# andrewcsmith/soundsym

Hardware: NVIDIA B200
Metric: dtw_cell_updates_per_s (higher is better)
Workload: dtype f16 (packed-half DP scan on f16 tensor-core costs; winners refined in f64)

## Files before the change

### soundsym_b200/csrc/dtw_h2.cu

```cuda
#include <algorithm>
#include <atomic>

#include "match.cuh"
#include "tc_common.cuh"

namespace ss {

int dtw_rescore_finalize(ss_dict* d, ss_queries* q, int k, int kp, uint32_t nslots, const uint32_t* d_slot_qid, double eps,
                         const float* d_max_na, const float* d_max_nb, const float* d_slot_max_na, int bound_mode, uint8_t* d_uncert_flag,
                         uint32_t* d_out_idx, double* d_out_dist);

int dtw_second_chance(ss_dict* d, ss_queries* q, int k, int kp, uint32_t nslots, const uint32_t* d_slot_qid, const unsigned long long* d_partial,
                      uint32_t nlists, const unsigned long long* d_thr, double eps, const float* d_max_na, const float* d_max_nb,
                      const float* d_slot_max_na, int bound_mode, uint8_t* d_uncert_flag, uint32_t* d_out_idx, double* d_out_dist);

constexpr int kH2Slots = 2;
constexpr int kH2SlotCols = 64;
constexpr int kH2DpWarps = 4 * kH2Slots;
constexpr int kH2DpThreads = kH2DpWarps * 32;
constexpr int kH2Threads = (kH2DpWarps + 1) * 32;
constexpr int kH2DescInt4 = 4;
constexpr int kH2In = 1, kH2Out = 2;
constexpr int kH2ARing = 32;
constexpr int kH2MaxLong = 2048;

struct H2Params {
    const unsigned char* a_blocks;
    const uint64_t* group_off;
    const uint32_t* group_len;
    const uint32_t* slot_len;
    uint32_t ngroups;
    const unsigned char* tiles;
    const int4* desc;
    const uint32_t* slice_tile;
    uint32_t nslices, slice_begin;
    unsigned long long* partial;
    uint32_t max_len;
    float inv_s;
    unsigned long long* thr;
    float* dbg;
    uint32_t dbg_nseg;
    __half2* bnd;
    uint32_t bnd_rows;
    float eta;
    unsigned long long* timeline;
};
__device__ __forceinline__ unsigned long long h2_now() {
    unsigned long long t;
    asm volatile("mov.u64 %0, %%globaltimer;" : "=l"(t));
    return t;
}

template <int N>
__device__ __forceinline__ void h2_ld(uint32_t taddr, __half2* v);
template <>
__device__ __forceinline__ void h2_ld<4>(uint32_t taddr, __half2* v) {
    uint32_t r[4];
    asm volatile("tcgen05.ld.sync.aligned.32x32b.x4.pack::16b.b32 {%0, %1, %2, %3}, [%4];\n" : "=r"(r[0]), "=r"(r[1]), "=r"(r[2]), "=r"(r[3]) : "r"(taddr));
#pragma unroll
    for (int i = 0; i < 4; i++) v[i] = *reinterpret_cast<__half2*>(&r[i]);
}
template <>
__device__ __forceinline__ void h2_ld<8>(uint32_t taddr, __half2* v) {
    uint32_t r[8];
    asm volatile("tcgen05.ld.sync.aligned.32x32b.x8.pack::16b.b32 {%0, %1, %2, %3, %4, %5, %6, %7}, [%8];\n"
                 : "=r"(r[0]), "=r"(r[1]), "=r"(r[2]), "=r"(r[3]), "=r"(r[4]), "=r"(r[5]), "=r"(r[6]), "=r"(r[7])
                 : "r"(taddr));
#pragma unroll
    for (int i = 0; i < 8; i++) v[i] = *reinterpret_cast<__half2*>(&r[i]);
}
template <>
__device__ __forceinline__ void h2_ld<16>(uint32_t taddr, __half2* v) {
    uint32_t r[16];
    asm volatile(
        "tcgen05.ld.sync.aligned.32x32b.x16.pack::16b.b32 {%0, %1, %2, %3, %4, %5, %6, %7, %8, %9, %10, %11, %12, %13, %14, %15}, [%16];\n"
        : "=r"(r[0]), "=r"(r[1]), "=r"(r[2]), "=r"(r[3]), "=r"(r[4]), "=r"(r[5]), "=r"(r[6]), "=r"(r[7]), "=r"(r[8]), "=r"(r[9]), "=r"(r[10]),
          "=r"(r[11]), "=r"(r[12]), "=r"(r[13]), "=r"(r[14]), "=r"(r[15])
        : "r"(taddr));
#pragma unroll
    for (int i = 0; i < 16; i++) v[i] = *reinterpret_cast<__half2*>(&r[i]);
}
template <int NG>
__device__ __forceinline__ void h2_ld_row(uint32_t taddr, __half2 (&v)[4 * NG]) {
    constexpr int N = 4 * NG;
    int done = 0;
    if constexpr (N >= 32) {
        h2_ld<16>(taddr, v);
        h2_ld<16>(taddr + 32, v + 16);
        done = 32;
    } else if constexpr (N >= 16) {
        h2_ld<16>(taddr, v);
        done = 16;
    }
    if constexpr ((N & 8) != 0) {
        h2_ld<8>(taddr + 2 * done, v + done);
        done += 8;
    }
    if constexpr ((N & 4) != 0) h2_ld<4>(taddr + 2 * done, v + done);
}

__device__ __forceinline__ __half2 h2_min3(__half2 a, __half2 b, __half2 c) { return __hmin2(__hmin2(a, b), c); }
__device__ __forceinline__ __half2 h2_inf() {
    const uint32_t bits = 0x7C007C00u;
    return *reinterpret_cast<const __half2*>(&bits);
}
__device__ __forceinline__ __half2 h2_zero() {
    const uint32_t bits = 0u;
    return *reinterpret_cast<const __half2*>(&bits);
}
__device__ __forceinline__ __half2 h2_combine(__half2 a, __half2 b) {
    const uint32_t r = __byte_perm(*reinterpret_cast<uint32_t*>(&a), *reinterpret_cast<uint32_t*>(&b), 0x7610);
    return *reinterpret_cast<const __half2*>(&r);
}
__device__ __forceinline__ int h2_len_of(const int4& sc, int e) { return (int)((((e < 4) ? (uint32_t)sc.x : (uint32_t)sc.y) >> (8 * (e & 3))) & 0xFFu); }
__device__ __forceinline__ int h2_seg_of(const int4& sa, const int4& sb, int e) {
    return e == 0 ? sa.x : e == 1 ? sa.y : e == 2 ? sa.z : e == 3 ? sa.w : e == 4 ? sb.x : e == 5 ? sb.y : e == 6 ? sb.z : sb.w;
}
__device__ __forceinline__ uint32_t h2_selp(uint32_t a, uint32_t b, int pick_a) {
    uint32_t r;
    asm("{\n.reg .pred q;\nsetp.ne.s32 q, %3, 0;\nselp.b32 %0, %1, %2, q;\n}\n" : "=r"(r) : "r"(a), "r"(b), "r"(pick_a));
    return r;
}
__device__ __forceinline__ __half2 h2_pick4(const __half2* v, int r) {
    const uint32_t v0 = *reinterpret_cast<const uint32_t*>(&v[0]), v1 = *reinterpret_cast<const uint32_t*>(&v[1]);
    const uint32_t v2 = *reinterpret_cast<const uint32_t*>(&v[2]), v3 = *reinterpret_cast<const uint32_t*>(&v[3]);
    const uint32_t lo = h2_selp(v1, v0, r & 1), hi = h2_selp(v3, v2, r & 1);
    const uint32_t o = h2_selp(hi, lo, r & 2);
    return *reinterpret_cast<const __half2*>(&o);
}

template <int NG>
__device__ __forceinline__ void h2_band(const __half2 (&tm0)[4 * NG], const __half2 (&tm1)[4 * NG], __half2 (&d)[4 * NG], __half2 dinit, __half2 (&c0l)[4]) {
    __half2 left0 = h2_inf(), diag0 = dinit, left1 = h2_inf();
#pragma unroll
    for (int j = 0; j < 4 * NG; j++) {
        const __half2 up0 = d[j];
        const __half2 c0 = __hadd2(tm0[j], h2_min3(left0, up0, diag0));
        const __half2 c1 = __hadd2(tm1[j], h2_min3(left1, c0, left0));
        diag0 = up0;
        left0 = c0;
        left1 = c1;
        d[j] = c1;
        if (j >= 4 * (NG - 1)) c0l[j - 4 * (NG - 1)] = c0;
    }
}
template <int NG>
__device__ __forceinline__ void h2_band_io(const __half2 (&tm0)[4 * NG], const __half2 (&tm1)[4 * NG], __half2 (&d)[4 * NG], __half2 l0, __half2 dg0,
                                           __half2 l1, __half2 (&c0l)[4], __half2& o0, __half2& o1) {
    __half2 left0 = l0, diag0 = dg0, left1 = l1;
#pragma unroll
    for (int j = 0; j < 4 * NG; j++) {
        const __half2 up0 = d[j];
        const __half2 c0 = __hadd2(tm0[j], h2_min3(left0, up0, diag0));
        const __half2 c1 = __hadd2(tm1[j], h2_min3(left1, c0, left0));
        diag0 = up0;
        left0 = c0;
        left1 = c1;
        d[j] = c1;
        if (j >= 4 * (NG - 1)) c0l[j - 4 * (NG - 1)] = c0;
    }
    o0 = left0, o1 = left1;
}
template <int NG>
__device__ __forceinline__ void h2_band_row_io(const __half2 (&tm)[4 * NG], __half2 (&d)[4 * NG], __half2 l0, __half2 dg0, __half2& o0) {
    __half2 left = l0, diag = dg0;
#pragma unroll
    for (int j = 0; j < 4 * NG; j++) {
        const __half2 up = d[j];
        const __half2 cur = __hadd2(tm[j], h2_min3(left, up, diag));
        diag = up;
        left = cur;
        d[j] = cur;
    }
    o0 = left;
}
template <int NG>
__device__ __forceinline__ void h2_band_row(const __half2 (&tm)[4 * NG], __half2 (&d)[4 * NG], __half2 dinit) {
    __half2 left = h2_inf(), diag = dinit;
#pragma unroll
    for (int j = 0; j < 4 * NG; j++) {
        const __half2 up = d[j];
        const __half2 cur = __hadd2(tm[j], h2_min3(left, up, diag));
        diag = up;
        left = cur;
        d[j] = cur;
    }
}

template <int NB, int NG>
__device__ __forceinline__ void h2_step2(TcCursor& cur, __half2 (&d)[NB][4 * NG], __half2 dinit, __half2 (&c0l)[NB][4]) {
    constexpr int kBandCols = kH2SlotCols / NB;
    cur.wait();
    const uint32_t taddr = cur.taddr;
    __half2 tm0[NB][4 * NG], tm1[NB][4 * NG];
#pragma unroll
    for (int b = 0; b < NB; b++) {
        h2_ld_row<NG>(taddr + b * kBandCols, tm0[b]);
        h2_ld_row<NG>(taddr + kTcN + b * kBandCols, tm1[b]);
    }
    tc_wait_ld();
    cur.release();
#pragma unroll
    for (int b = 0; b < NB; b++) h2_band<NG>(tm0[b], tm1[b], d[b], dinit, c0l[b]);
}

template <int NB, int NG>
__device__ __forceinline__ void h2_tile(uint32_t L, uint32_t lmin, uint32_t Lm, const int4& sc, TcCursor& cur, __half2 (&res)[NB]) {
    __half2 d[NB][4 * NG];
#pragma unroll
    for (int b = 0; b < NB; b++) {
#pragma unroll
        for (int j = 0; j < 4 * NG; j++) d[b][j] = h2_inf();
        res[b] = h2_inf();
    }
    __half2 dinit = h2_zero();
    const uint32_t nfull = L >> 1;
    const uint32_t ncap = min((lmin - 1) >> 1, nfull);
    uint32_t st = 0;
    if (st < ncap && cur.buf) {
        __half2 c0l[NB][4];
        h2_step2<NB, NG>(cur, d, dinit, c0l);
        dinit = h2_inf();
        st++;
    }
    if (st + 2 <= ncap) {
        const uint32_t full0 = cur.full, taddr0 = cur.taddr;
        uint32_t par = cur.par;
#pragma unroll 1
        for (; st + 2 <= ncap; st += 2) {
            __half2 c0l[NB][4];
            TcCursor c0 = {0u, par, full0, taddr0, cur.full_sum, cur.taddr_sum};
            h2_step2<NB, NG>(c0, d, dinit, c0l);
            TcCursor c1 = {1u, par, full0 + 8u, taddr0 + (uint32_t)kTcBufCols, cur.full_sum, cur.taddr_sum};
            h2_step2<NB, NG>(c1, d, h2_inf(), c0l);
            dinit = h2_inf();
            par ^= 1u;
        }
        cur.par = par;
    }
    if (st < ncap) {
        __half2 c0l[NB][4];
        h2_step2<NB, NG>(cur, d, dinit, c0l);
        dinit = h2_inf();
        st++;
    }
#pragma unroll 1
    for (; st < nfull; st++) {
        __half2 c0l[NB][4];
        h2_step2<NB, NG>(cur, d, dinit, c0l);
        dinit = h2_inf();
        const bool end0 = 2 * st + 1 == Lm, end1 = 2 * st + 2 == Lm;
#pragma unroll
        for (int b = 0; b < NB; b++) {
            const int ra = (h2_len_of(sc, 2 * b) - 1) & 3, rb = (h2_len_of(sc, 2 * b + 1) - 1) & 3;
            const __half2 e0 = h2_combine(h2_pick4(c0l[b], ra), h2_pick4(c0l[b], rb));
            const __half2 e1 = h2_combine(h2_pick4(&d[b][4 * (NG - 1)], ra), h2_pick4(&d[b][4 * (NG - 1)], rb));
            res[b] = end0 ? e0 : (end1 ? e1 : res[b]);
        }
    }
    if (L & 1) {
        constexpr int kBandCols = kH2SlotCols / NB;
        cur.wait();
        __half2 tm0[NB][4 * NG];
#pragma unroll
        for (int b = 0; b < NB; b++) h2_ld_row<NG>(cur.taddr + b * kBandCols, tm0[b]);
        tc_wait_ld();
        cur.release();
#pragma unroll
        for (int b = 0; b < NB; b++) {
            h2_band_row<NG>(tm0[b], d[b], dinit);
            const int ra = (h2_len_of(sc, 2 * b) - 1) & 3, rb = (h2_len_of(sc, 2 * b + 1) - 1) & 3;
            const __half2 e = h2_combine(h2_pick4(&d[b][4 * (NG - 1)], ra), h2_pick4(&d[b][4 * (NG - 1)], rb));
            res[b] = (L == Lm) ? e : res[b];
        }
    }
}

template <int NG, bool IN, bool OUT>
__device__ __forceinline__ void h2_tile_strip(uint32_t L, uint32_t lmin, uint32_t Lm, const int4& sc, TcCursor& cur, __half2* bnd, __half2& res) {
    constexpr uint32_t kStride = kH2DpThreads;
    __half2 d[4 * NG];
#pragma unroll
    for (int j = 0; j < 4 * NG; j++) d[j] = h2_inf();
    res = h2_inf();
    __half2 prev_b = IN ? h2_inf() : h2_zero();
    const uint32_t nfull = L >> 1;
    const uint32_t ncap = OUT ? nfull : min((lmin - 1) >> 1, nfull);
    const int ra = (h2_len_of(sc, 0) - 1) & 3, rb = (h2_len_of(sc, 1) - 1) & 3;
#pragma unroll 1
    for (uint32_t st = 0; st < nfull; st++) {
        __half2 b0 = h2_inf(), b1 = h2_inf();
        if (IN) b0 = bnd[(size_t)(2 * st) * kStride], b1 = bnd[(size_t)(2 * st + 1) * kStride];
        cur.wait();
        const uint32_t taddr = cur.taddr;
        __half2 tm0[4 * NG], tm1[4 * NG], c0l[4], o0, o1;
        h2_ld_row<NG>(taddr, tm0);
        h2_ld_row<NG>(taddr + kTcN, tm1);
        tc_wait_ld();
        cur.release();
        h2_band_io<NG>(tm0, tm1, d, b0, prev_b, b1, c0l, o0, o1);
        prev_b = IN ? b1 : h2_inf();
        if (OUT) {
            bnd[(size_t)(2 * st) * kStride] = o0;
            bnd[(size_t)(2 * st + 1) * kStride] = o1;
        } else if (st >= ncap) {
            const bool end0 = 2 * st + 1 == Lm, end1 = 2 * st + 2 == Lm;
            const __half2 e0 = h2_combine(h2_pick4(c0l, ra), h2_pick4(c0l, rb));
            const __half2 e1 = h2_combine(h2_pick4(&d[4 * (NG - 1)], ra), h2_pick4(&d[4 * (NG - 1)], rb));
            res = end0 ? e0 : (end1 ? e1 : res);
        }
    }
    if (L & 1) {
        __half2 b0 = h2_inf();
        if (IN) b0 = bnd[(size_t)(L - 1) * kStride];
        cur.wait();
        __half2 tm0[4 * NG], o0;
        h2_ld_row<NG>(cur.taddr, tm0);
        tc_wait_ld();
        cur.release();
        h2_band_row_io<NG>(tm0, d, b0, prev_b, o0);
        if (OUT) {
            bnd[(size_t)(L - 1) * kStride] = o0;
        } else {
            const __half2 e = h2_combine(h2_pick4(&d[4 * (NG - 1)], ra), h2_pick4(&d[4 * (NG - 1)], rb));
            res = (L == Lm) ? e : res;
        }
    }
// ... 97 lines not shown
#pragma unroll
        for (int s = 0; s < KP; s++) list[s * kH2DpThreads] = 0xFFFFFFFFFFFFFFFFull;
        const unsigned long long thr0 = __ldcg(p.thr + g * kTcM + m);
        unsigned long long worst = thr0;
        int cnt = 0, wpos = 0;
        const uint32_t lane_addr = tmem_base + ((uint32_t)(q * 32) << 16) + slot * kH2SlotCols;
        const uint32_t Lm = p.slot_len[g * kTcM + m];
        TcCursor cur;
        cur.init(s32(t_full), lane_addr);
        const int4* dp = p.desc + ((size_t)t0 * kH2Slots + slot) * kH2DescInt4;
        int4 na = make_int4(0, 0, 0, 0), nb = na, nc = na;
        if (ntiles) na = __ldg(dp), nb = __ldg(dp + 1), nc = __ldg(dp + 2);
        for (uint32_t n = 0; n < ntiles; n++) {
            const int4 sa = na, sb = nb, sc = nc;
            dp += kH2Slots * kH2DescInt4;
            if (n + 1 < ntiles) na = __ldg(dp), nb = __ldg(dp + 1), nc = __ldg(dp + 2);
            const int ng = sc.z;
            __half2 res[NB];
            if constexpr (NB == 1) {
                switch (ng) {
                    case 5: h2_tile<1, 5>(L, lmin, Lm, sc, cur, res); break;
                    case 6: h2_tile<1, 6>(L, lmin, Lm, sc, cur, res); break;
                    case 7: h2_tile<1, 7>(L, lmin, Lm, sc, cur, res); break;
                    default: h2_tile<1, 8>(L, lmin, Lm, sc, cur, res); break;
                }
            } else if constexpr (NB == 2) {
                if (ng == 3) h2_tile<2, 3>(L, lmin, Lm, sc, cur, res);
                else h2_tile<2, 4>(L, lmin, Lm, sc, cur, res);
            } else {
                if (ng == 1) h2_tile<4, 1>(L, lmin, Lm, sc, cur, res);
                else h2_tile<4, 2>(L, lmin, Lm, sc, cur, res);
            }
            if (tl && threadIdx.x == 0 && n + 1 == (ntiles + 1) / 2) tl[6] = h2_now();
            if (Lm) {
#pragma unroll
                for (int b = 0; b < NB; b++) {
#pragma unroll
                    for (int hsel = 0; hsel < 2; hsel++) {
                        const int e = 2 * b + hsel;
                        const int seg = h2_seg_of(sa, sb, e);
                        if (seg >= 0) {
                            const float v = hsel ? __high2float(res[b]) : __low2float(res[b]);
                            const float dist = __fdividef(v * p.inv_s, (float)(Lm + (uint32_t)h2_len_of(sc, e)));
                            const unsigned long long key = ((unsigned long long)tc_f2ord(dist) << 32) | (uint32_t)seg;
                            if (key < worst && dist == dist) {
                                const bool full = cnt == KP;
                                list[(full ? wpos : cnt) * kH2DpThreads] = key;
                                cnt += full ? 0 : 1;
                                if (cnt == KP) {
                                    tc_list_max<KP, kH2DpThreads>(list, worst, wpos);
                                    worst = worst < thr0 ? worst : thr0;
                                }
                            }
                            if constexpr (DBG) p.dbg[(size_t)(g * kTcM + m) * p.dbg_nseg + seg] = dist;
                        }
                    }
                }
            }
        }
        tc_sort_list<KP, kH2DpThreads>(list, cnt);
        worst = list[(KP - 1) * kH2DpThreads];
        worst = worst < thr0 ? worst : thr0;
        asm volatile("bar.sync 1, %0;" ::"n"(kH2DpThreads) : "memory");
        if (tl && threadIdx.x == 0) tl[2] = h2_now(), tl[5] = clock64() - tl[5];
        if (slot == 0) {
            const unsigned long long* other = list + kTcM;
            for (int s = 0; s < KP; s++) {
                const unsigned long long key = other[s * kH2DpThreads];
                if (key >= worst) break;
                tc_insert_key<KP, kH2DpThreads>(list, worst, key);
                worst = worst < thr0 ? worst : thr0;
            }
            const unsigned long long kept_worst = list[(KP - 1) * kH2DpThreads];
            if (kept_worst != 0xFFFFFFFFFFFFFFFFull && kept_worst < thr0) atomicMin(p.thr + g * kTcM + m, kept_worst);
            unsigned long long* out = p.partial + ((size_t)slice * p.ngroups * kTcM + (size_t)g * kTcM + m) * KP;
#pragma unroll
            for (int s = 0; s < KP; s++) out[s] = list[s * kH2DpThreads];
        }
    }
    if constexpr (NB != 1) asm volatile("griddepcontrol.wait;" ::: "memory");
    tc_fence_before();
    __syncthreads();
    if (warp == kH2DpWarps) {
        tc_fence_after();
        asm volatile("tcgen05.dealloc.cta_group::1.sync.aligned.b32 %0, %1;" ::"r"(tmem_base), "r"(512u) : "memory");
    }
    if (tl && threadIdx.x == 0) tl[3] = h2_now();
}

template <int KP, int NB, bool DBG = false>
__global__ void __launch_bounds__(kH2Threads, 1) k_dtw_scan_h2_long(const H2Params p) {
    extern __shared__ unsigned char smem_raw[];
    unsigned char* smem = smem_raw + ((128u - (s32(smem_raw) & 127u)) & 127u);
    unsigned char* sA = smem;
    unsigned char* sB = smem + (size_t)kH2ARing * kTcATileBytes;
    uint64_t* bars = reinterpret_cast<uint64_t*>(sB + kTcStages * kTcBTileBytes);
    uint64_t* a_full = bars;
    uint64_t* a_empty = bars + 4;
    uint64_t* b_full = bars + 8;
    uint64_t* b_empty = bars + 12;
    uint64_t* t_full = bars + 16;
    uint64_t* t_empty = bars + 18;
    uint32_t* tmem_slot = reinterpret_cast<uint32_t*>(bars + 20);
    unsigned long long* topk = reinterpret_cast<unsigned long long*>(bars + 32);

    const int warp = threadIdx.x >> 5, lane = threadIdx.x & 31;
    const uint32_t g = blockIdx.x / p.nslices, slice = p.slice_begin + blockIdx.x % p.nslices;
    asm volatile("griddepcontrol.launch_dependents;" ::: "memory");
    const uint32_t glen = p.group_len[g];
    const uint32_t L = glen & 0xFFFFu, lmin = glen >> 16;
    const uint32_t t0 = p.slice_tile[slice], t1 = p.slice_tile[slice + 1];
    const uint32_t ntiles = t1 - t0;

    if (threadIdx.x == 0) {
        for (int s = 0; s < 4; s++) mb_init(&a_full[s], 1), mb_init(&a_empty[s], 1);
        for (int s = 0; s < kTcStages; s++) mb_init(&b_full[s], 1), mb_init(&b_empty[s], 1);
        for (int s = 0; s < 2; s++) mb_init(&t_full[s], 1), mb_init(&t_empty[s], kH2DpWarps);
        asm volatile("fence.mbarrier_init.release.cluster;" ::: "memory");
    }
    if (warp == kH2DpWarps) {
        asm volatile("tcgen05.alloc.cta_group::1.sync.aligned.shared::cta.b32 [%0], %1;" ::"r"(s32(tmem_slot)), "r"(512u) : "memory");
        asm volatile("tcgen05.relinquish_alloc_permit.cta_group::1.sync.aligned;" ::: "memory");
    }
    tc_fence_before();
    __syncthreads();
    tc_fence_after();
    const uint32_t tmem_base = *tmem_slot;
    if (warp == kH2DpWarps) {
        if (lane == 0 && ntiles) {
            const uint32_t bars_s = s32(bars), sA_s = s32(sA), sB_s = s32(sB);
            const uint32_t a_full_s = bars_s, a_empty_s = bars_s + 32, b_full_s = bars_s + 64, b_empty_s = bars_s + 96, t_full_s = bars_s + 128,
                           t_empty_s = bars_s + 144;
            const uint32_t npieces = (L + 7) >> 3;
            const bool streaming = npieces > 4;
            const uint32_t total_pieces = streaming ? ntiles * npieces : npieces;
            const unsigned char* a_src = p.a_blocks + p.group_off[g];
            auto load_piece = [&](uint32_t n) {
                const uint32_t pc = n % npieces, slot = streaming ? (n & 3u) : pc;
                const uint32_t rows = min(8u, L - 8u * pc);
                mbs_expect_tx(a_full_s + 8 * slot, rows * kTcATileBytes);
                tmas_g2s(sA_s + slot * 8 * kTcATileBytes, a_src + (size_t)pc * 8 * kTcATileBytes, rows * kTcATileBytes, a_full_s + 8 * slot);
            };
            for (uint32_t n = 0; n < total_pieces && n < 4; n++) load_piece(n);
            const unsigned char* tile_src = p.tiles + (size_t)t0 * kTcBTileBytes;
            for (uint32_t n = 0; n < ntiles && n < (uint32_t)kTcStages; n++) {
                mbs_expect_tx(b_full_s + 8 * n, kTcBTileBytes);
                tmas_g2s(sB_s + n * kTcBTileBytes, tile_src + (size_t)n * kTcBTileBytes, kTcBTileBytes, b_full_s + 8 * n);
            }
            tile_src += (size_t)kTcStages * kTcBTileBytes;
            const uint32_t idesc = (0u << 4) | ((uint32_t)(kTcN >> 3) << 17) | ((uint32_t)(kTcM >> 4) << 24);
            uint32_t cnt = 0, stage = 0, sphase = 0, use_n = 0;
            for (uint32_t n = 0; n < ntiles; n++) {
                mbs_wait_sleep(b_full_s + 8 * stage, sphase);
                const uint64_t bdesc = tc_smem_desc_s<kTcN>(sB_s + stage * kTcBTileBytes);
                for (uint32_t pc = 0; pc < npieces; pc++, use_n++) {
                    const uint32_t slot = streaming ? (use_n & 3u) : pc;
                    if (streaming && use_n >= 1 && use_n + 3 < total_pieces) {
                        mbs_wait_sleep(a_empty_s + 8 * ((use_n - 1) & 3u), ((use_n - 1) >> 2) & 1);
                        load_piece(use_n + 3);
                    }
                    if (streaming || n == 0) mbs_wait_sleep(a_full_s + 8 * slot, streaming ? ((use_n >> 2) & 1) : 0u);
                    const uint64_t adesc0 = tc_smem_desc_s<kTcM>(sA_s + slot * 8 * kTcATileBytes);
                    const uint32_t rows = min(8u, L - 8u * pc);
                    for (uint32_t r = 0; r < rows; r += 2, cnt++) {
                        const uint32_t buf = cnt & 1;
                        if (cnt >= 2) mbs_wait_sleep(t_empty_s + 8 * buf, ((cnt >> 1) - 1) & 1);
// ... 229 lines not shown
        for (int slot = 0; slot < kH2Slots; slot++) {
            int segs[8] = {-1, -1, -1, -1, -1, -1, -1, -1}, whole[4] = {0, 0, 0, 0};
            uint32_t lens[2] = {0, 0};
            for (int e = 0; e < 2 * nb; e++) {
                const size_t pos = (size_t)slot * 2 * nb + e;
                if (pos < take) {
                    segs[e] = (int)order[o + pos];
                    lens[e >> 2] |= (uint32_t)len_of(order[o + pos]) << (8 * (e & 3));
                    if (e < 4) whole[e] = len_of(order[o + pos]);
                }
            }
            desc.push_back(make_int4(segs[0], segs[1], segs[2], segs[3]));
            desc.push_back(make_int4(segs[4], segs[5], segs[6], segs[7]));
            desc.push_back(make_int4((int)lens[0], (int)lens[1], ng, 0));
            desc.push_back(make_int4(whole[0], whole[1], whole[2], whole[3]));
        }
        push_tile(nb, ng, (24u + 16u * (uint32_t)(nb * ng)) * (nb == 4 ? 3u : 2u) / 2u, false);
        o += take;
    }
    while (cur_kind < 4) {
        d->h2_first_tile[cur_kind == 1 ? 1 : 2] = (uint32_t)tile_nb.size();
        cur_kind *= 2;
    }
    d->h2_first_tile[3] = (uint32_t)tile_nb.size();
    const uint32_t ntiles = (uint32_t)tile_nb.size();
    d->h2_ntiles = ntiles;
    d->h2_slices.clear();
    if (!ntiles) return SS_OK;
    SS_TRY(upload(ctx, d->d_h2_desc, desc.data(), desc.size()));
    DevBuf<uint8_t> d_nb;
    SS_TRY(upload(ctx, d_nb, tile_nb.data(), tile_nb.size()));
    SS_CUDA(ctx, d->d_h2_tiles.reserve((size_t)ntiles * kTcBTileBytes / 2));
    k_h2_dict_tiles<<<ntiles, kTcN, 0, ctx->stream>>>(d->d_mfcc.p, d->d_off.p, d->c, d->d_mu.p, d->d_h2_desc.p, d_nb.p, ntiles, d->tc_nb_scale,
                                                     reinterpret_cast<unsigned char*>(d->d_h2_tiles.p));
    SS_LAUNCHED(ctx);
    SS_CUDA(ctx, cudaStreamSynchronize(ctx->stream));
    float S = 1.0f;
    while (S * d->tc_max_nb > 4096.f) S *= 0.5f;
    while (S * d->tc_max_nb < 2048.f && S < 64.f) S *= 2.0f;
    d->h2_s0 = S;
    d->h2_s = S;
    d->h2_bmax = d->tc_max_abs;
    {
        DevBuf<uint32_t> d_n;
        SS_CUDA(ctx, d_n.reserve(1));
        k_h2_nsmid<<<1, 1, 0, ctx->stream>>>(d_n.p);
        SS_LAUNCHED(ctx);
        SS_CUDA(ctx, cudaMemcpyAsync(&d->h2_nsmid, d_n.p, sizeof(uint32_t), cudaMemcpyDeviceToHost, ctx->stream));
        SS_CUDA(ctx, cudaStreamSynchronize(ctx->stream));
    }
    d->h2_ready = true;
    return SS_OK;
}

static void h2_cost_scale(ss_dict* d, const ss_queries* q) {
    float S = d->h2_s0;
    for (uint64_t l = 64; l < (uint64_t)d->max_len + q->max_len && S > 1.0f / 65536.f; l *= 2) S *= 0.5f;
    d->h2_s = S;
}

static int h2_queries_build(ss_dict* d, ss_queries* q) {
    ss_ctx* ctx = q->ctx;
    h2_cost_scale(d, q);
    if (q->h2_built && q->h2_dict_serial == d->tc_serial && q->h2_s_built == d->h2_s) return SS_OK;
    if (!q->tc_grouped) SS_TRY(dtw_tc_queries_group(q));
    SS_CUDA(ctx, q->d_h2_a.reserve(std::max<uint64_t>(q->tc_a_bytes, 16)));
    SS_CUDA(ctx, q->d_tc_slot_max_na.reserve(std::max<size_t>((size_t)q->tc_ngroups * kTcM, 1)));
    SS_CUDA(ctx, q->d_uncert_flag.reserve(std::max<size_t>(q->nq, 1)));
    SS_CUDA(ctx, q->d_tc_max_norm.reserve(1));
    SS_CUDA(ctx, cudaMemsetAsync(q->d_tc_max_norm.p, 0, sizeof(float), ctx->stream));
    if (q->tc_ngroups) {
        SS_CUDA(ctx, cudaMemsetAsync(q->d_tc_slot_max_na.p, 0, (size_t)q->tc_ngroups * kTcM * sizeof(float), ctx->stream));
        k_tc_query_tiles<<<dim3(q->tc_ngroups, q->max_len), kTcM, 0, ctx->stream>>>(q->d_mfcc.p, q->d_off.p, q->c, d->d_mu.p, q->d_tc_group_len.p,
                                                                 q->d_tc_group_off.p, q->d_tc_qid.p, d->tc_nb_scale, d->h2_s, q->d_h2_a.p,
                                                                 q->d_tc_max_norm.p, q->d_tc_slot_max_na.p);
        SS_LAUNCHED(ctx);
    }
    q->h2_built = true;
    q->h2_dict_serial = d->tc_serial;
    q->h2_s_built = d->h2_s;
    return SS_OK;
}

template <int KP, int NB, bool DBG, bool LONG>
static int h2_launch_kind(ss_ctx* ctx, H2Params p, uint32_t slice_begin, uint32_t nslices, size_t smem, bool dependent) {
    if (!nslices) return SS_OK;
    p.slice_begin = slice_begin;
    p.nslices = nslices;
    auto kern = LONG ? k_dtw_scan_h2_long<KP, NB, DBG> : k_dtw_scan_h2<KP, NB, DBG>;
    SS_CUDA(ctx, cudaFuncSetAttribute(kern, cudaFuncAttributeMaxDynamicSharedMemorySize, (int)smem));
    cudaLaunchConfig_t cfg = {};
    cfg.gridDim = dim3(p.ngroups * nslices);
    cfg.blockDim = dim3(kH2Threads);
    cfg.dynamicSmemBytes = smem;
    cfg.stream = ctx->stream;
    cudaLaunchAttribute attr[1];
    attr[0].id = cudaLaunchAttributeProgrammaticStreamSerialization;
    attr[0].val.programmaticStreamSerializationAllowed = 1;
    cfg.attrs = attr;
    cfg.numAttrs = dependent ? 1 : 0;
    SS_CUDA(ctx, cudaLaunchKernelEx(&cfg, kern, p));
    SS_LAUNCHED(ctx);
    return SS_OK;
}

static double h2_eta(const ss_dict* d) { return (13.0 * (double)d->h2_bmax + 4.0) * 5.9604644775390625e-08  / (double)d->h2_s; }

struct H2Plan {
    H2Params p;
    uint32_t kind_begin[4];
    uint32_t nslots;
    size_t smem;
    bool use_long;
};
constexpr int kH2Waves = 16;
constexpr int kH2Kp = 8;

static int h2_plan(ss_dict* d, ss_queries* q, int kp, H2Plan* plan) {
    ss_ctx* ctx = d->ctx;
    const uint32_t nslots = q->tc_ngroups * kTcM;
    if (d->h2_slices.size() > 64 && !d->h2_slices.count(q->tc_ngroups)) {
        SS_CUDA(ctx, cudaStreamSynchronize(ctx->stream));
        d->h2_slices.clear();
    }
    std::unique_ptr<ss_dict::H2Slices>& sl = d->h2_slices[q->tc_ngroups];
    if (!sl) {
        sl.reset(new ss_dict::H2Slices());
        const uint32_t want = std::max<uint32_t>(1, std::min<uint32_t>(((uint32_t)ctx->sm_count * kH2Waves + q->tc_ngroups - 1) / q->tc_ngroups,
                                                                       std::max<uint32_t>((uint32_t)ctx->sm_count, d->h2_ntiles / 12)));
        std::vector<uint32_t> st;
        uint64_t total = 0;
        for (uint32_t f : d->h_h2_tile_cost) total += f;
        const uint64_t per0 = std::max<uint64_t>(1, (total + want - 1) / want);
        int last_kind = -1, nkinds = 0;
        for (int kind = 0; kind < 3; kind++)
            if (d->h2_first_tile[kind + 1] > d->h2_first_tile[kind]) last_kind = kind, nkinds++;
        if (nkinds < 2) last_kind = -1;
        for (int kind = 0; kind < 3; kind++) {
            sl->kind_slice[kind] = (uint32_t)st.size();
            const uint64_t per = kind == last_kind ? std::max<uint64_t>(1, per0 / 2) : per0;
            uint64_t acc = per;
            for (uint32_t t = d->h2_first_tile[kind]; t < d->h2_first_tile[kind + 1]; t++) {
                if (acc >= per && !d->h_h2_tile_cont[t]) st.push_back(t), acc = 0;
                acc += d->h_h2_tile_cost[t];
            }
        }
        sl->kind_slice[3] = (uint32_t)st.size();
        st.push_back(d->h2_ntiles);
        SS_TRY(upload(ctx, sl->d_slice_tile, st.data(), st.size()));
    }
    const uint32_t nslices = sl->kind_slice[3];
    SS_CUDA(ctx, d->d_tc_partial.reserve((size_t)nslices * nslots * kp));
    SS_CUDA(ctx, d->d_cand_idx.reserve((size_t)nslots * kp));
    SS_CUDA(ctx, d->d_cand_adist.reserve((size_t)nslots * kp));
    if (!d->ev_scan0) {
        SS_CUDA(ctx, cudaEventCreate(&d->ev_scan0));
        SS_CUDA(ctx, cudaEventCreate(&d->ev_scan1));
    }
    H2Params& p = plan->p;
    p.a_blocks = q->d_h2_a.p;
    p.group_off = q->d_tc_group_off.p;
    p.group_len = q->d_tc_group_len.p;
    p.slot_len = q->d_tc_slot_len.p;
    p.ngroups = q->tc_ngroups;
    p.tiles = reinterpret_cast<const unsigned char*>(d->d_h2_tiles.p);
    p.desc = d->d_h2_desc.p;
    p.slice_tile = sl->d_slice_tile.p;
    p.nslices = nslices;
    p.slice_begin = 0;
    p.partial = d->d_tc_partial.p;
    p.max_len = q->max_len;
    p.inv_s = 1.0f / d->h2_s;
    SS_CUDA(ctx, d->d_h2_thr.reserve(std::max<uint32_t>(nslots, 1)));
    SS_CUDA(ctx, cudaMemsetAsync(d->d_h2_thr.p, 0xFF, (size_t)nslots * sizeof(unsigned long long), ctx->stream));
    p.thr = d->d_h2_thr.p;
    p.dbg = nullptr;
    p.dbg_nseg = 0;
    for (int i = 0; i < 4; i++) plan->kind_begin[i] = sl->kind_slice[i];
    plan->nslots = nslots;
    plan->use_long = d->h2_has_strips || q->max_len > (uint32_t)kTcMaxLen;
    p.bnd = nullptr;
    p.bnd_rows = 0;
    p.eta = 0.f;
    p.timeline = nullptr;
    if (plan->use_long) {
        if (d->h2_has_strips) {
            p.bnd_rows = (q->max_len + 1) & ~1u;
            SS_CUDA(ctx, d->d_h2_bnd.reserve((size_t)d->h2_nsmid * p.bnd_rows * kH2DpThreads));
            p.bnd = d->d_h2_bnd.p;
        }
        p.eta = (float)h2_eta(d) * 1.0001f;
        plan->smem = (size_t)kH2ARing * kTcATileBytes + kTcStages * kTcBTileBytes + 32 * 8 + (size_t)kp * kH2DpThreads * 8 + 1024;
    } else {
        plan->smem = (size_t)q->max_len * kTcATileBytes + kTcStages * kTcBTileBytes + 32 * 8 + (size_t)kp * kH2DpThreads * 8 + 1024;
    }
    return SS_OK;
}

template <int KP, bool DBG, bool LONG>
// ... 93 lines not shown
```

Before: 9146 billion.

## Add two-pipe H2 DTW scan kernel with split TMEM loads and register rebalancing

Adds a new kernel variant that runs two independent MMA/DP pipelines per CTA. Each pipeline has its own producer warp, B-tile stages and TMEM buffer, and the tiles of a slice are interleaved across the two pipes. DP warps now use a simple single-buffer cursor. Their TMEM row loads are split so the first half of the band is computed while the second half is still loading, and the buffer is released earlier. setmaxnreg shifts registers from producer warps to DP warps. The kernel is chosen for KP=8 with NB of 1 or 2. It aims to hide MMA and TMEM-load latency behind the scalar half2 DP recurrence, at the cost of more threads, more shared memory and a per-CTA merge of more top-k lists.

Measured after the change: 10250 billion, median of 6. 12.1% higher.

```diff
diff --git a/soundsym_b200/csrc/dtw_h2.cu b/soundsym_b200/csrc/dtw_h2.cu
--- a/soundsym_b200/csrc/dtw_h2.cu
+++ b/soundsym_b200/csrc/dtw_h2.cu
@@ -1,5 +1,6 @@
 #include <algorithm>
 #include <atomic>
+#include <type_traits>
 
 #include "match.cuh"
 #include "tc_common.cuh"
@@ -23,6 +24,12 @@
 constexpr int kH2In = 1, kH2Out = 2;
 constexpr int kH2ARing = 32;
 constexpr int kH2MaxLong = 2048;
+constexpr int kH2Pipes = 2;
+constexpr int kH2PDpWarps = kH2Pipes * kH2DpWarps;
+constexpr int kH2PDpThreads = kH2PDpWarps * 32;
+constexpr int kH2PThreads = (kH2PDpWarps + 4) * 32;
+constexpr int kH2PRegsDp = 112, kH2PRegsProd = 32;
+static_assert(kH2PDpThreads * kH2PRegsDp + 128 * kH2PRegsProd == kH2PThreads * 96, "setmaxnreg budget must match the launch pool");
 
 struct H2Params {
     const unsigned char* a_blocks;
@@ -187,25 +194,95 @@
     }
 }
 
-template <int NB, int NG>
-__device__ __forceinline__ void h2_step2(TcCursor& cur, __half2 (&d)[NB][4 * NG], __half2 dinit, __half2 (&c0l)[NB][4]) {
+template <int NG, int J0, int J1>
+__device__ __forceinline__ void h2_band_cols(const __half2* tm0, const __half2* tm1, __half2 (&d)[4 * NG], __half2& left0, __half2& diag0,
+                                             __half2& left1, __half2 (&c0l)[4]) {
+#pragma unroll
+    for (int j = J0; j < J1; j++) {
+        const __half2 up0 = d[j];
+        const __half2 c0 = __hadd2(tm0[j - J0], h2_min3(left0, up0, diag0));
+        const __half2 c1 = __hadd2(tm1[j - J0], h2_min3(left1, c0, left0));
+        diag0 = up0;
+        left0 = c0;
+        left1 = c1;
+        d[j] = c1;
+        if (j >= 4 * (NG - 1)) c0l[j - 4 * (NG - 1)] = c0;
+    }
+}
+
+struct H2PipeCursor {
+    uint32_t par, full, taddr;
+    __device__ __forceinline__ void wait() const {
+        mb_wait_addr(full, par);
+        tc_fence_after();
+    }
+    __device__ __forceinline__ void release() {
+        tc_fence_before();
+        mb_arrive_elect(full + 16);
+        par ^= 1u;
+    }
+};
+
+template <int NB, int NG, class Cur>
+__device__ __forceinline__ void h2_step2(Cur& cur, __half2 (&d)[NB][4 * NG], __half2 dinit, __half2 (&c0l)[NB][4]) {
     constexpr int kBandCols = kH2SlotCols / NB;
     cur.wait();
     const uint32_t taddr = cur.taddr;
-    __half2 tm0[NB][4 * NG], tm1[NB][4 * NG];
-#pragma unroll
-    for (int b = 0; b < NB; b++) {
-        h2_ld_row<NG>(taddr + b * kBandCols, tm0[b]);
-        h2_ld_row<NG>(taddr + kTcN + b * kBandCols, tm1[b]);
-    }
-    tc_wait_ld();
-    cur.release();
-#pragma unroll
-    for (int b = 0; b < NB; b++) h2_band<NG>(tm0[b], tm1[b], d[b], dinit, c0l[b]);
-}
-
-template <int NB, int NG>
-__device__ __forceinline__ void h2_tile(uint32_t L, uint32_t lmin, uint32_t Lm, const int4& sc, TcCursor& cur, __half2 (&res)[NB]) {
+    if constexpr (std::is_same<Cur, H2PipeCursor>::value && NB == 1) {
+        static_assert(NG >= 5, "NB = 1 tiles have 5..8 column groups");
+        __half2 left0 = h2_inf(), diag0 = dinit, left1 = h2_inf();
+        {
+            __half2 a0[16], a1[16];
+            h2_ld_row<4>(taddr, a0);
+            h2_ld_row<4>(taddr + kTcN, a1);
+            tc_wait_ld();
+            h2_band_cols<NG, 0, 16>(a0, a1, d[0], left0, diag0, left1, c0l[0]);
+        }
+        __half2 b0[4 * (NG - 4)], b1[4 * (NG - 4)];
+        h2_ld_row<NG - 4>(taddr + 32, b0);
+        h2_ld_row<NG - 4>(taddr + kTcN + 32, b1);
+        tc_wait_ld();
+        cur.release();
+        h2_band_cols<NG, 16, 4 * NG>(b0, b1, d[0], left0, diag0, left1, c0l[0]);
+    } else if constexpr (std::is_same<Cur, H2PipeCursor>::value) {
+        constexpr int H = NB / 2;
+        {
+            __half2 tm0[H][4 * NG], tm1[H][4 * NG];
+#pragma unroll
+            for (int b = 0; b < H; b++) {
+                h2_ld_row<NG>(taddr + b * kBandCols, tm0[b]);
+                h2_ld_row<NG>(taddr + kTcN + b * kBandCols, tm1[b]);
+            }
+            tc_wait_ld();
+#pragma unroll
+            for (int b = 0; b < H; b++) h2_band<NG>(tm0[b], tm1[b], d[b], dinit, c0l[b]);
+        }
+        __half2 tm0[H][4 * NG], tm1[H][4 * NG];
+#pragma unroll
+        for (int b = 0; b < H; b++) {
+            h2_ld_row<NG>(taddr + (H + b) * kBandCols, tm0[b]);
+            h2_ld_row<NG>(taddr + kTcN + (H + b) * kBandCols, tm1[b]);
+        }
+        tc_wait_ld();
+        cur.release();
+#pragma unroll
+        for (int b = 0; b < H; b++) h2_band<NG>(tm0[b], tm1[b], d[H + b], dinit, c0l[H + b]);
+    } else {
+        __half2 tm0[NB][4 * NG], tm1[NB][4 * NG];
+#pragma unroll
+        for (int b = 0; b < NB; b++) {
+            h2_ld_row<NG>(taddr + b * kBandCols, tm0[b]);
+            h2_ld_row<NG>(taddr + kTcN + b * kBandCols, tm1[b]);
+        }
+        tc_wait_ld();
+        cur.release();
+#pragma unroll
+        for (int b = 0; b < NB; b++) h2_band<NG>(tm0[b], tm1[b], d[b], dinit, c0l[b]);
+    }
+}
+
+template <int NB, int NG, class Cur>
+__device__ __forceinline__ void h2_tile(uint32_t L, uint32_t lmin, uint32_t Lm, const int4& sc, Cur& cur, __half2 (&res)[NB]) {
     __half2 d[NB][4 * NG];
 #pragma unroll
     for (int b = 0; b < NB; b++) {
@@ -217,32 +294,41 @@
     const uint32_t nfull = L >> 1;
     const uint32_t ncap = min((lmin - 1) >> 1, nfull);
     uint32_t st = 0;
-    if (st < ncap && cur.buf) {
-        __half2 c0l[NB][4];
-        h2_step2<NB, NG>(cur, d, dinit, c0l);
-        dinit = h2_inf();
-        st++;
-    }
-    if (st + 2 <= ncap) {
-        const uint32_t full0 = cur.full, taddr0 = cur.taddr;
-        uint32_t par = cur.par;
+    if constexpr (std::is_same<Cur, H2PipeCursor>::value) {
 #pragma unroll 1
-        for (; st + 2 <= ncap; st += 2) {
+        for (; st < ncap; st++) {
             __half2 c0l[NB][4];
-            TcCursor c0 = {0u, par, full0, taddr0, cur.full_sum, cur.taddr_sum};
-            h2_step2<NB, NG>(c0, d, dinit, c0l);
-            TcCursor c1 = {1u, par, full0 + 8u, taddr0 + (uint32_t)kTcBufCols, cur.full_sum, cur.taddr_sum};
-            h2_step2<NB, NG>(c1, d, h2_inf(), c0l);
+            h2_step2<NB, NG>(cur, d, dinit, c0l);
             dinit = h2_inf();
-            par ^= 1u;
-        }
-        cur.par = par;
-    }
-    if (st < ncap) {
-        __half2 c0l[NB][4];
-        h2_step2<NB, NG>(cur, d, dinit, c0l);
-        dinit = h2_inf();
-        st++;
+        }
+    } else {
+        if (st < ncap && cur.buf) {
+            __half2 c0l[NB][4];
+            h2_step2<NB, NG>(cur, d, dinit, c0l);
+            dinit = h2_inf();
+            st++;
+        }
+        if (st + 2 <= ncap) {
+            const uint32_t full0 = cur.full, taddr0 = cur.taddr;
+            uint32_t par = cur.par;
+#pragma unroll 1
+            for (; st + 2 <= ncap; st += 2) {
+                __half2 c0l[NB][4];
+                TcCursor c0 = {0u, par, full0, taddr0, cur.full_sum, cur.taddr_sum};
+                h2_step2<NB, NG>(c0, d, dinit, c0l);
+                TcCursor c1 = {1u, par, full0 + 8u, taddr0 + (uint32_t)kTcBufCols, cur.full_sum, cur.taddr_sum};
+                h2_step2<NB, NG>(c1, d, h2_inf(), c0l);
+                dinit = h2_inf();
+                par ^= 1u;
+            }
+            cur.par = par;
+        }
+        if (st < ncap) {
+            __half2 c0l[NB][4];
+            h2_step2<NB, NG>(cur, d, dinit, c0l);
+            dinit = h2_inf();
+            st++;
+        }
     }
 #pragma unroll 1
     for (; st < nfull; st++) {
@@ -506,6 +592,195 @@
     tc_fence_before();
     __syncthreads();
     if (warp == kH2DpWarps) {
+        tc_fence_after();
+        asm volatile("tcgen05.dealloc.cta_group::1.sync.aligned.b32 %0, %1;" ::"r"(tmem_base), "r"(512u) : "memory");
+    }
+    if (tl && threadIdx.x == 0) tl[3] = h2_now();
+}
+
+template <int KP, int NB, bool DBG = false>
+__global__ void __launch_bounds__(kH2PThreads, 1) k_dtw_scan_h2_2p(const H2Params p) {
+    extern __shared__ unsigned char smem_raw[];
+    unsigned char* smem = smem_raw + ((128u - (s32(smem_raw) & 127u)) & 127u);
+    unsigned char* sA = smem;
+    unsigned char* sB = smem + (size_t)p.max_len * kTcATileBytes;
+    uint64_t* bars = reinterpret_cast<uint64_t*>(sB + kH2Pipes * kTcStages * kTcBTileBytes);
+    uint64_t* a_full = bars;
+    uint64_t* t_full = bars + 1 + 2 * kH2Pipes * kTcStages;
+    uint64_t* t_empty = t_full + kH2Pipes;
+    uint32_t* tmem_slot = reinterpret_cast<uint32_t*>(t_empty + kH2Pipes);
+    unsigned long long* topk = reinterpret_cast<unsigned long long*>(bars + 32);
+
+    const int warp = threadIdx.x >> 5, lane = threadIdx.x & 31;
+    uint32_t g, slice;
+    if (blockIdx.x < p.ngroups) {
+        g = blockIdx.x, slice = p.slice_begin;
+    } else {
+        const uint32_t r = blockIdx.x - p.ngroups;
+        g = r / (p.nslices - 1), slice = p.slice_begin + 1 + r % (p.nslices - 1);
+    }
+    asm volatile("griddepcontrol.launch_dependents;" ::: "memory");
+    const uint32_t glen = p.group_len[g];
+    const uint32_t L = glen & 0xFFFFu, lmin = glen >> 16;
+    const uint32_t t0 = p.slice_tile[slice], t1 = p.slice_tile[slice + 1];
+    const uint32_t ntiles = t1 - t0;
+    unsigned long long* tl = p.timeline ? p.timeline + ((size_t)(p.slice_begin * p.ngroups) + blockIdx.x) * 8 : nullptr;
+    if (tl && threadIdx.x == 0) {
+        unsigned smid;
+        asm("mov.u32 %0, %%smid;" : "=r"(smid));
+        tl[0] = h2_now(), tl[4] = smid | ((unsigned long long)NB << 16) | ((unsigned long long)g << 32), tl[7] = ((unsigned long long)L << 32) | ntiles;
+    }
+
+    if (threadIdx.x == 0) {
+        mb_init(a_full, 1);
+        for (int s = 0; s < 2 * kH2Pipes * kTcStages; s++) mb_init(&bars[1 + s], 1);
+        for (int s = 0; s < kH2Pipes; s++) mb_init(&t_full[s], 1), mb_init(&t_empty[s], kH2DpWarps);
+        asm volatile("fence.mbarrier_init.release.cluster;" ::: "memory");
+    }
+    if (warp == kH2PDpWarps) {
+        asm volatile("tcgen05.alloc.cta_group::1.sync.aligned.shared::cta.b32 [%0], %1;" ::"r"(s32(tmem_slot)), "r"(512u) : "memory");
+        asm volatile("tcgen05.relinquish_alloc_permit.cta_group::1.sync.aligned;" ::: "memory");
+    }
+    tc_fence_before();
+    __syncthreads();
+    tc_fence_after();
+    const uint32_t tmem_base = *tmem_slot;
+    if (tl && threadIdx.x == 0) tl[1] = h2_now(), tl[5] = clock64();
+    if (warp >= kH2PDpWarps) {
+        asm volatile("setmaxnreg.dec.sync.aligned.u32 %0;" ::"n"(kH2PRegsProd));
+        const uint32_t pipe = (uint32_t)(warp - kH2PDpWarps);
+        const uint32_t ntp = ntiles > pipe ? (ntiles - pipe + 1) >> 1 : 0u;
+        if (pipe < (uint32_t)kH2Pipes && lane == 0 && ntp) {
+            const uint32_t bars_s = s32(bars), sA_s = s32(sA), sB_s = s32(sB) + pipe * (kTcStages * kTcBTileBytes);
+            const uint32_t a_full_s = bars_s, b_full_s = bars_s + 8 + pipe * (16 * kTcStages), b_empty_s = b_full_s + 8 * kTcStages,
+                           t_full_s = s32(t_full) + 8 * pipe, t_empty_s = t_full_s + 16;
+            if (pipe == 0) {
+                mbs_expect_tx(a_full_s, L * kTcATileBytes);
+                tmas_g2s(sA_s, p.a_blocks + p.group_off[g], L * kTcATileBytes, a_full_s);
+            }
+            constexpr size_t kStride = (size_t)kH2Pipes * kTcBTileBytes;
+            const unsigned char* tile_src = p.tiles + (size_t)(t0 + pipe) * kTcBTileBytes;
+            for (uint32_t n = 0; n < ntp && n < (uint32_t)kTcStages; n++) {
+                mbs_expect_tx(b_full_s + 8 * n, kTcBTileBytes);
+                tmas_g2s(sB_s + n * kTcBTileBytes, tile_src + n * kStride, kTcBTileBytes, b_full_s + 8 * n);
+            }
+            tile_src += kTcStages * kStride;
+            mbs_wait_sleep(a_full_s, 0);
+            const uint32_t idesc = (0u << 4) | ((uint32_t)(kTcN >> 3) << 17) | ((uint32_t)(kTcM >> 4) << 24);
+            const uint64_t adesc0 = tc_smem_desc_s<kTcM>(sA_s);
+            const uint32_t tm = tmem_base + pipe * kTcBufCols;
+            uint32_t cnt = 0, stage = 0, sphase = 0;
+            for (uint32_t n = 0; n < ntp; n++) {
+                mbs_wait_sleep(b_full_s + 8 * stage, sphase);
+                const uint64_t bdesc = tc_smem_desc_s<kTcN>(sB_s + stage * kTcBTileBytes);
+                uint64_t adesc = adesc0;
+                for (uint32_t row = 0; row < L; row += 2, cnt++) {
+                    if (cnt >= 1) mbs_wait_sleep(t_empty_s, (cnt - 1) & 1);
+                    tc_fence_after();
+                    tc_mma_f16(tm, adesc, bdesc, idesc);
+                    if (row + 1 < L) tc_mma_f16(tm + kTcN, adesc + (kTcATileBytes >> 4), bdesc, idesc);
+                    tcs_commit(t_full_s);
+                    adesc += 2 * (kTcATileBytes >> 4);
+                }
+                tcs_commit(b_empty_s + 8 * stage);
+                if (n + kTcStages < ntp) {
+                    mbs_wait_sleep(b_empty_s + 8 * stage, sphase);
+                    mbs_expect_tx(b_full_s + 8 * stage, kTcBTileBytes);
+                    tmas_g2s(sB_s + stage * kTcBTileBytes, tile_src, kTcBTileBytes, b_full_s + 8 * stage);
+                    tile_src += kStride;
+                }
+                if (++stage == (uint32_t)kTcStages) stage = 0, sphase ^= 1;
+            }
+        }
+    } else {
+        asm volatile("setmaxnreg.inc.sync.aligned.u32 %0;" ::"n"(kH2PRegsDp));
+        const int q = warp & 3, slot = (warp >> 2) & 1, pipe = warp >> 3;
+        const int m = q * 32 + lane;
+        unsigned long long* list = topk + threadIdx.x;
+#pragma unroll
+        for (int s = 0; s < KP; s++) list[s * kH2PDpThreads] = 0xFFFFFFFFFFFFFFFFull;
+        const unsigned long long thr0 = __ldcg(p.thr + g * kTcM + m);
+        unsigned long long worst = thr0;
+        int cnt = 0, wpos = 0;
+        const uint32_t Lm = p.slot_len[g * kTcM + m];
+        H2PipeCursor cur = {0u, s32(t_full + pipe), tmem_base + ((uint32_t)(q * 32) << 16) + (uint32_t)(pipe * kTcBufCols + slot * kH2SlotCols)};
+        const uint32_t ntp = ntiles > (uint32_t)pipe ? (ntiles - pipe + 1) >> 1 : 0u;
+        const int4* dp = p.desc + ((size_t)(t0 + pipe) * kH2Slots + slot) * kH2DescInt4;
+        int4 na = make_int4(0, 0, 0, 0), nb = na, nc = na;
+        if (ntp) na = __ldg(dp), nb = __ldg(dp + 1), nc = __ldg(dp + 2);
+        for (uint32_t n = 0; n < ntp; n++) {
+            const int4 sa = na, sb = nb, sc = nc;
+            dp += kH2Pipes * kH2Slots * kH2DescInt4;
+            if (n + 1 < ntp) na = __ldg(dp), nb = __ldg(dp + 1), nc = __ldg(dp + 2);
+            const int ng = sc.z;
+            __half2 res[NB];
+            if constexpr (NB == 1) {
+                switch (ng) {
+                    case 5: h2_tile<1, 5>(L, lmin, Lm, sc, cur, res); break;
+                    case 6: h2_tile<1, 6>(L, lmin, Lm, sc, cur, res); break;
+                    case 7: h2_tile<1, 7>(L, lmin, Lm, sc, cur, res); break;
+                    default: h2_tile<1, 8>(L, lmin, Lm, sc, cur, res); break;
+                }
+            } else if constexpr (NB == 2) {
+                if (ng == 3) h2_tile<2, 3>(L, lmin, Lm, sc, cur, res);
+                else h2_tile<2, 4>(L, lmin, Lm, sc, cur, res);
+            } else {
+                if (ng == 1) h2_tile<4, 1>(L, lmin, Lm, sc, cur, res);
+                else h2_tile<4, 2>(L, lmin, Lm, sc, cur, res);
+            }
+            if (tl && threadIdx.x == 0 && n + 1 == (ntp + 1) / 2) tl[6] = h2_now();
+            if (Lm) {
+#pragma unroll
+                for (int b = 0; b < NB; b++) {
+#pragma unroll
+                    for (int hsel = 0; hsel < 2; hsel++) {
+                        const int e = 2 * b + hsel;
+                        const int seg = h2_seg_of(sa, sb, e);
+                        if (seg >= 0) {
+                            const float v = hsel ? __high2float(res[b]) : __low2float(res[b]);
+                            const float dist = __fdividef(v * p.inv_s, (float)(Lm + (uint32_t)h2_len_of(sc, e)));
+                            const unsigned long long key = ((unsigned long long)tc_f2ord(dist) << 32) | (uint32_t)seg;
+                            if (key < worst && dist == dist) {
+                                const bool full = cnt == KP;
+                                list[(full ? wpos : cnt) * kH2PDpThreads] = key;
+                                cnt += full ? 0 : 1;
+                                if (cnt == KP) {
+                                    tc_list_max<KP, kH2PDpThreads>(list, worst, wpos);
+                                    worst = worst < thr0 ? worst : thr0;
+                                }
+                            }
+                            if constexpr (DBG) p.dbg[(size_t)(g * kTcM + m) * p.dbg_nseg + seg] = dist;
+                        }
+                    }
+                }
+            }
+        }
+        tc_sort_list<KP, kH2PDpThreads>(list, cnt);
+        worst = list[(KP - 1) * kH2PDpThreads];
+        worst = worst < thr0 ? worst : thr0;
+        asm volatile("bar.sync 1, %0;" ::"n"(kH2PDpThreads) : "memory");
+        if (tl && threadIdx.x == 0) tl[2] = h2_now(), tl[5] = clock64() - tl[5];
+        if (threadIdx.x < kTcM) {
+            for (int o = 1; o < kH2Pipes * kH2Slots; o++) {
+                const unsigned long long* other = list + o * kTcM;
+                for (int s = 0; s < KP; s++) {
+                    const unsigned long long key = other[s * kH2PDpThreads];
+                    if (key >= worst) break;
+                    tc_insert_key<KP, kH2PDpThreads>(list, worst, key);
+                    worst = worst < thr0 ? worst : thr0;
+                }
+            }
+            const unsigned long long kept_worst = list[(KP - 1) * kH2PDpThreads];
+            if (kept_worst != 0xFFFFFFFFFFFFFFFFull && kept_worst < thr0) atomicMin(p.thr + g * kTcM + m, kept_worst);
+            unsigned long long* out = p.partial + ((size_t)slice * p.ngroups * kTcM + (size_t)g * kTcM + m) * KP;
+#pragma unroll
+            for (int s = 0; s < KP; s++) out[s] = list[s * kH2PDpThreads];
+        }
+    }
+    if constexpr (NB != 1) asm volatile("griddepcontrol.wait;" ::: "memory");
+    tc_fence_before();
+    __syncthreads();
+    if (warp == kH2PDpWarps) {
         tc_fence_after();
         asm volatile("tcgen05.dealloc.cta_group::1.sync.aligned.b32 %0, %1;" ::"r"(tmem_base), "r"(512u) : "memory");
     }
@@ -901,16 +1176,28 @@
     return SS_OK;
 }
 
+constexpr int kH2Kp = 8;
+
 template <int KP, int NB, bool DBG, bool LONG>
 static int h2_launch_kind(ss_ctx* ctx, H2Params p, uint32_t slice_begin, uint32_t nslices, size_t smem, bool dependent) {
     if (!nslices) return SS_OK;
     p.slice_begin = slice_begin;
     p.nslices = nslices;
-    auto kern = LONG ? k_dtw_scan_h2_long<KP, NB, DBG> : k_dtw_scan_h2<KP, NB, DBG>;
+    void (*kern)(H2Params);
+    unsigned threads = kH2Threads;
+    if constexpr (LONG) {
+        kern = k_dtw_scan_h2_long<KP, NB, DBG>;
+    } else if constexpr (KP == kH2Kp && NB != 4) {
+        kern = k_dtw_scan_h2_2p<KP, NB, DBG>;
+        threads = kH2PThreads;
+        smem = (size_t)p.max_len * kTcATileBytes + kH2Pipes * kTcStages * kTcBTileBytes + 32 * 8 + (size_t)KP * kH2PDpThreads * 8 + 1024;
+    } else {
+        kern = k_dtw_scan_h2<KP, NB, DBG>;
+    }
     SS_CUDA(ctx, cudaFuncSetAttribute(kern, cudaFuncAttributeMaxDynamicSharedMemorySize, (int)smem));
     cudaLaunchConfig_t cfg = {};
     cfg.gridDim = dim3(p.ngroups * nslices);
-    cfg.blockDim = dim3(kH2Threads);
+    cfg.blockDim = dim3(threads);
     cfg.dynamicSmemBytes = smem;
     cfg.stream = ctx->stream;
     cudaLaunchAttribute attr[1];
@@ -933,7 +1220,6 @@
     bool use_long;
 };
 constexpr int kH2Waves = 16;
-constexpr int kH2Kp = 8;
 
 static int h2_plan(ss_dict* d, ss_queries* q, int kp, H2Plan* plan) {
     ss_ctx* ctx = d->ctx;
```
